# XiaoshuiHuang/IMFNet

Measured on AMD Instinct MI355X. Metric: descriptors/sec (32-D) on 3DMatch fragments, higher is better.
Workload: dtype f32 (bf16x3)

## Files before the change

### imfnet_amd/_lib.py

```python
import ctypes as C
import os

_HERE = os.path.dirname(os.path.abspath(__file__))
LIB_PATH = os.environ.get("IMF_LIB") or os.path.join(_HERE, "libimfnet_hip.so")

TILE_ROWS = 64
MASK_WORDS = 4
MAX_KVOL = 125
MAX_BATCH = 8
FLAG_RANGE = 32
XYZ_F32_QUOTIENT = 2
TAG_LABEL, TAG_REGS, TAG_WAVE8, TAG_WAVE4, TAG_HEAD, TAG_HALF, TAG_U48, TAG_OCC = 1, 2, 4, 8, 16, 64, 128, 256


class ImfError(RuntimeError):
    pass


class ConvArgs(C.Structure):
    _fields_ = [
        ("in_a", C.c_void_p), ("in_b", C.c_void_p),
        ("c_a", C.c_int32), ("c_b", C.c_int32),
        ("w_packed", C.c_void_p),
        ("kvol", C.c_int32), ("cout", C.c_int32),
# ... 219 lines not shown
    "imf_graph_end_capture": (_I, [_P, C.POINTER(C.c_void_p), C.POINTER(C.c_int)]),
    "imf_graph_abort_capture": (_I, [_P]),
    "imf_graph_launch": (_I, [_P, _P]),
    "imf_graph_destroy": (None, [_P]),
    "imf_pyramid_arena_bytes_caps": (_Z, [_L, _I, C.POINTER(C.c_int64)]),
    "imf_pyramid_build_dyn": (_I, [_P, _I, _P, _L, C.POINTER(C.c_int64), _D, _I, _P, _Z, _P, C.POINTER(LevelDesc), _P]),
    "imf_rulebook_conv_dyn": (_I, [_P, _L, _P, _L, _P, _I, _I, _P, _P, _P, _P]),
    "imf_rulebook_transpose_dyn": (_I, [_P, _L, _P, _L, _P, _I, _I, _P, _P, _P, _L, _P, _P]),
    "imf_conv_first_bitgrid_dyn": (_I, [_P, _L, _P, _P, _P, _I, _P, _Z, _P, _I, _P, _P, _I, _P, _P]),
    "imf_fusion_workspace_bytes_cap": (_Z, [_L]),
    "imf_fusion_attention_dyn": (_I, [_P, _L, _P, _P, _I, _P, C.POINTER(C.c_void_p), C.POINTER(C.c_void_p), _I, _I,
                                      C.POINTER(FusionWeights), C.c_float, _P, _P, _Z, _P]),
    "imf_fusion_attention_dyn_v": (_I, [_P, _L, _P, _P, _I, _P, C.POINTER(C.c_void_p), C.POINTER(C.c_void_p), _I, _I,
                                        C.POINTER(FusionWeights), C.c_float, _P, _P, _Z, _I, _P]),
    "imf_host_rigid_fit": (_I, [_P, _P, _I, _P]),
    "imf_ransac_workspace_bytes": (_Z, [_I]),
    "imf_ransac_registration": (_I, [_P, _L, _P, _L, _P, _I, _D, _D, _I, C.c_uint64, _P, _P, _P, _P, _Z, _P]),
    "imf_gather_points": (_I, [_P, _I, _P, _P, _L, _P, _P]),
    "imf_icp_workspace_bytes": (_Z, [_L, _L]),
    "imf_icp_point_to_point": (_I, [_P, _L, _P, _L, _D, _P, _I, _P, _P, _P, _P, _Z, _P]),
    "imf_icp_plane_workspace_bytes": (_Z, [_L, _L]),
    "imf_icp_point_to_plane": (_I, [_P, _L, _P, _P, _L, _D, _P, _I, _P, _P, _P, _P, _Z, _P]),
    "imf_normals_workspace_bytes": (_Z, [_L]),
    "imf_estimate_normals": (_I, [_P, _L, _I, _D, _P, _P, _P, _P, _P, _P, _Z, _P]),
    "imf_radius_count_workspace_bytes": (_Z, [_L]),
    "imf_radius_count": (_I, [_P, _L, _P, _L, _P, _D, _P, _P, _P, _P, _Z, _P]),
    "imf_radius_pairs_workspace_bytes": (_Z, [_L, _L]),
    "imf_radius_pairs": (_I, [_P, _L, _P, _L, _P, _D, _P, _P, _L, _P, _P, _P, _Z, _P]),
    "imf_robust_transform_workspace_bytes": (_Z, [_L]),
    "imf_robust_transform": (_I, [_P, _P, _P, _L, _P, _P, _P, _Z, _P]),
    "imf_tsdf_allocate_workspace_bytes": (_Z, [_L]),
    "imf_tsdf_allocate": (_I, [_P, _I, _P, C.POINTER(TsdfParams), _I, _P, _L, _P, _L, _P, _P, _Z, _P]),
    "imf_tsdf_integrate": (_I, [_P, _I, _P, C.POINTER(TsdfParams), _P, _P, _L, _P, _P]),
    "imf_tsdf_extract_workspace_bytes": (_Z, [_L]),
    "imf_tsdf_extract": (_I, [_P, _P, _P, _L, _P, _L, C.POINTER(TsdfParams), _P, _L, _P, _P, _Z, _P]),
    "imf_overlap_index_bytes": (_Z, [_L]),
    "imf_overlap_index_workspace_bytes": (_Z, [_L]),
    "imf_overlap_index_build": (_I, [_P, _L, _D, _P, _Z, C.POINTER(OverlapIndex), _P, _Z, _P]),
    "imf_overlap_bound": (_I, [_P, _P, _I, _L, _P, _P]),
    "imf_overlap_pair": (_I, [C.POINTER(OverlapIndex), C.POINTER(OverlapIndex), C.c_float, _L, _P, _P]),
    "imf_overlap_emit_workspace_bytes": (_Z, [_L]),
    "imf_overlap_emit": (_I, [_P, _L, _P, _P, _P, _Z, _P]),
    "imf_hash_capacity": (_L, [_L]),
    "imf_unique_workspace_bytes": (_Z, [_L]),
    "imf_voxelize": (_I, [_P, _I, _L, _D, _I, _P, _P, _P, _P, _L, _P, _P, _P]),
    "imf_downsample": (_I, [_P, _P, _L, _I, _P, _P, _P, _L, _P, _P]),
    "imf_pyramid_arena_bytes": (_Z, [_L, _I]),
    "imf_pyramid_build": (_I, [_P, _I, _L, _D, _I, _I, _P, _Z, _P, C.POINTER(LevelDesc), _P]),
    "imf_pyramid_build_batched": (_I, [_P, _I, _L, _D, C.POINTER(C.c_int64), _I, _I, _P, _Z, _P,
                                       C.POINTER(LevelDesc), _P]),
    "imf_rulebook_slots": (_L, [_L]),
    "imf_rulebook_conv": (_I, [_P, _L, _P, _L, _I, _I, _P, _P, _P, _P]),
    "imf_rulebook_sorted_workspace_bytes": (C.c_size_t, [_L]),
    "imf_rulebook_sort_by_occupancy": (_I, [_P, _I, _L, _L, _P, _P, _P, _P, _P, C.c_size_t, _P]),
    "imf_resunet_sorted_maps": (_I, [_I]),
    "imf_resunet_sorted_maps_n": (_I, [_I, _I]),
    "imf_rulebook_transpose_slots": (_L, [_L]),
    "imf_rulebook_transpose": (_I, [_P, _L, _P, _L, _I, _I, _P, _P, _P, _L, _P, _P]),
    "imf_packed_weight_floats": (_L, [_I, _I, _I]),
    "imf_packed_weight_floats_split16": (_L, [_I, _I, _I]),
    "imf_pack_weights": (_I, [_P, _I, _I, _I, _P, _P]),
    "imf_first_kernel_image_floats": (_L, [_I, _I]),
    "imf_pack_first_kernel": (_I, [_P, _I, _I, _P, _P]),
    "imf_pack_weights_split16": (_I, [_P, _I, _I, _I, _P, _P]),
    "imf_packed_weight_floats_bf16x3": (_L, [_I, _I, _I]),
    "imf_pack_weights_bf16x3": (_I, [_P, _I, _I, _I, _P, _P]),
    "imf_spconv_auto_split": (_I, [_L, _I, _I]),
    "imf_spconv_workspace_bytes": (_Z, [_L, _I, _I]),
    "imf_spconv_fwd": (_I, [C.POINTER(ConvArgs), _P]),
    "imf_pointwise_head": (_I, [C.POINTER(HeadArgs), _P]),
    "imf_spconv_small_cin": (_I, [_P, _I, _P, _I, _I, _P, _L, _L, _P, _P, _I, _P, _P]),
    "imf_fusion_workspace_bytes": (_Z, [_L]),
    "imf_fusion_attention_batched": (_I, [_P, _I, C.POINTER(C.c_int64), C.POINTER(C.c_int64), C.POINTER(C.c_void_p),
                                          C.POINTER(C.c_void_p), _I, _I, C.POINTER(FusionWeights), C.c_float, _P, _P,
                                          _Z, _P]),
    "imf_fusion_attention": (_I, [_P, _L, _P, _P, _I, _I, C.POINTER(FusionWeights), C.c_float, _P, _P, _Z, _P]),
    "imf_fusion_attention_batched_v": (_I, [_P, _I, C.POINTER(C.c_int64), C.POINTER(C.c_int64), C.POINTER(C.c_void_p),
                                            C.POINTER(C.c_void_p), _I, _I, C.POINTER(FusionWeights), C.c_float, _P, _P,
                                            _Z, _P, _I, _P]),
    "imf_image_workspace_bytes": (_Z, [_I, _I, _I]),
    "imf_image_tokens": (_I, [_I, _I]),
    "imf_image_tables_build": (_I, [_I, _I, _I, _P, _Z, _P]),
    "imf_image_branch": (_I, [C.POINTER(ImageDesc), _P, _I, _I, _I, _P, _Z, _P, _P, _P, _I, _P, _P]),
    "imf_image_train_tables_bytes": (_Z, [_I, _I, _I]),
    "imf_image_train_tables_build": (_I, [_I, _I, _I, _P, _Z, C.POINTER(ImageTrainTables), _P]),
    "imf_image_im2col7": (_I, [_P, _I, _I, _I, _P, _P]),
    "imf_image_maxpool_forward": (_I, [_P, _I, _I, _I, _I, _P, _P, _P]),
    "imf_image_maxpool_backward": (_I, [_P, _P, _I, _I, _I, _I, _P, _P]),
    "imf_conv_first_bitgrid_flags": (_I, [_P, _L, _P, _I, _P, _Z, _P, _I, _P, _P, _I, _P, _P, _P]),
    "imf_fusion_attention_batched_flags": (_I, [_P, _I, C.POINTER(C.c_int64), C.POINTER(C.c_int64), C.POINTER(C.c_void_p),
                                                C.POINTER(C.c_void_p), _I, _I, C.POINTER(FusionWeights), C.c_float, _P, _P,
                                                _Z, _P, _P]),
    "imf_bitgrid_words": (_Z, [_P, _I]),
    "imf_conv_first_bitgrid": (_I, [_P, _L, _P, _I, _P, _Z, _P, _I, _P, _P, _I, _P, _P]),
    "imf_conv_first_fused": (_I, [_P, _L, _P, _L, _I, _I, _P, _I, _P, _I, _P, _P, _I, _P, _P]),
}

_lib = None


def lib():
    global _lib
    if _lib is None:
        if not os.path.exists(LIB_PATH):
            raise ImfError(
                f"{LIB_PATH} not found: build it with `python -c 'import __graft_entry__ as g; g.build()'` "
                "or `make -C imfnet_amd/csrc`.  imfnet_amd has no CPU fallback.")
        handle = C.CDLL(LIB_PATH)
        for name, (res, args) in SIGNATURES.items():
            fn = getattr(handle, name)
            fn.restype, fn.argtypes = res, args
        _lib = handle
    return _lib


def check(rc, what):
    if rc != 0:
        msg = lib().imf_last_error().decode("utf-8", "replace")
        raise ImfError(f"{what} failed (rc={rc}): {msg}")
```

### imfnet_amd/csrc/image.hip

```cpp
#include <stdio.h>
#include <stdlib.h>
#include <string.h>

#include "common.h"
#include "image_shared.h"

namespace imf {
namespace {

constexpr int kC1 = 64, kC2 = 128, kKV = 256;

struct Plan {
  Table t4, t48, td, t8;
  float *im2col, *stem, *b4[3], *b8[4], *ln, *kv, *splitk;
  size_t splitk_bytes, total_bytes, table_bytes;
};

size_t splitk_need(int64_t n_out, int cout, int kvol) {
  const int64_t n_slots = imf_rulebook_slots(n_out);
  return imf_spconv_workspace_bytes(n_slots, cout, imf_spconv_auto_split(n_slots, cout, kvol));
}

Plan plan_of(const ImgShape &s, void *ws) {
  Plan p;
// ... 108 lines not shown
}

}
}

using namespace imf;

extern "C" {

size_t imf_image_workspace_bytes(int B, int H, int W) {
  if (B < 1 || H < 8 || W < 8) return 0;
  return plan_of(shape_of(B, H, W), nullptr).total_bytes + 256;
}

int imf_image_tokens(int H, int W) {
  const ImgShape s = shape_of(1, H, W);
  return s.H8 * s.W8;
}

int imf_image_tables_build(int B, int H, int W, void *workspace, size_t workspace_bytes, void *stream) {
  IMF_REQUIRE(workspace && B >= 1 && B <= IMF_MAX_BATCH && H >= 8 && W >= 8, "imf_image_tables_build: bad argument");
  IMF_REQUIRE(((uintptr_t)workspace & 255) == 0, "imf_image_tables_build: workspace must be 256-byte aligned");
  IMF_REQUIRE(workspace_bytes >= imf_image_workspace_bytes(B, H, W), "imf_image_tables_build: workspace too small");
  const ImgShape s = shape_of(B, H, W);
  const Plan p = plan_of(s, workspace);
  hipStream_t st = (hipStream_t)stream;
  IMF_CHECK_HIP(hipMemsetAsync(workspace, 0, p.table_bytes, st));
  auto build = [&](const Table &t, int Hin, int Win, int Hout, int Wout, int ksize, int stride, int pad) {
    k_img_rulebook<<<(unsigned)div_up(t.n_slots * t.kvol, 256), 256, 0, st>>>(
        s.B, Hin, Win, Hout, Wout, ksize, stride, pad, t.n_slots, t.tile_rows, t.nbr, t.tile_mask);
  };
  build(p.t4, s.H4, s.W4, s.H4, s.W4, 3, 1, 1);
  build(p.t48, s.H4, s.W4, s.H8, s.W8, 3, 2, 1);
  build(p.td, s.H4, s.W4, s.H8, s.W8, 1, 2, 0);
  build(p.t8, s.H8, s.W8, s.H8, s.W8, 3, 1, 1);
  IMF_CHECK_LAUNCH("k_img_rulebook");
  return IMF_OK;
}

int imf_image_branch(const imf_image_desc *net, const float *image, int B, int H, int W, void *workspace,
                     size_t workspace_bytes, float *feat_out, float *kt_packed, float *v_packed,
                     int tokens_padded, int32_t *flags, void *stream) {
  IMF_REQUIRE(net && image && workspace, "imf_image_branch: null pointer");
  IMF_REQUIRE(B >= 1 && B <= IMF_MAX_BATCH && H >= 8 && W >= 8, "imf_image_branch: B=%d H=%d W=%d", B, H, W);
  IMF_REQUIRE(((uintptr_t)workspace & 255) == 0, "imf_image_branch: workspace must be 256-byte aligned");
  IMF_REQUIRE(workspace_bytes >= imf_image_workspace_bytes(B, H, W), "imf_image_branch: workspace too small");
  IMF_REQUIRE(net->stem_w && net->stem_scale && net->stem_shift, "imf_image_branch: stem weights missing");
  for (int i = 0; i < 15; ++i)
    IMF_REQUIRE(net->conv[i].w_packed && net->conv[i].scale && net->conv[i].shift, "imf_image_branch: conv %d missing", i);
  const ImgShape s = shape_of(B, H, W);
  const int ntok = s.H8 * s.W8;
  const bool want_kv = kt_packed || v_packed;
  if (want_kv) {
    IMF_REQUIRE(kt_packed && v_packed && net->ln_g && net->ln_b && net->kv_w, "imf_image_branch: K/V outputs need ln / kv weights");
    IMF_REQUIRE(tokens_padded % 64 == 0 && tokens_padded >= ntok, "imf_image_branch: tokens_padded=%d for %d tokens",
                tokens_padded, ntok);
  }
  const Plan p = plan_of(s, workspace);
  hipStream_t st = (hipStream_t)stream;

  auto conv = [&](const imf_net_conv &c, const Table *t, int64_t n_rows, const float *in, const float *residual,
                  float *out) -> int {
    imf_conv_args a;
    memset(&a, 0, sizeof(a));
    a.in_a = in; a.c_a = c.cin; a.w_packed = c.w_packed; a.kvol = c.kvol; a.cout = c.cout;
    if (t) {
      IMF_REQUIRE(t->kvol == c.kvol, "imf_image_branch: kernel volume %d on a %d-tap table", c.kvol, t->kvol);
      a.tile_rows = t->tile_rows; a.nbr = t->nbr; a.tile_mask = t->tile_mask;
      a.n_slots = t->n_slots; a.n_out = t->n_out;
    } else {
      a.n_slots = imf_rulebook_slots(n_rows); a.n_out = n_rows;
    }
    a.scale = c.scale; a.shift = c.shift; a.residual = residual; a.relu = c.relu; a.out = out;
    a.variant = c.variant; a.split_k = 0;
    a.dyn_err = c.variant == 6 ? flags : nullptr;
    a.kernel_tag = IMF_TAG_LABEL;
    if (c.kvol == 9 && (c.variant == 6 || c.variant == 0 || c.variant == 3) && c.cout % 64 == 0) {
      a.kernel_tag |= IMF_TAG_WAVE8;
      a.split_k = 1;
    }
    a.workspace = p.splitk; a.workspace_bytes = p.splitk_bytes;
    return imf_spconv_fwd(&a, st);
  };

  {
    const int64_t total = s.n2 * kStemK;
    k_img_im2col7<<<(unsigned)div_up(total, 256), 256, 0, st>>>(image, B, H, W, s.H2, s.W2, p.im2col, net->variant == 6 ? flags : nullptr);
    IMF_CHECK_LAUNCH("k_img_im2col7");
    imf_net_conv c;
    memset(&c, 0, sizeof(c));
    c.w_packed = net->stem_w; c.kvol = 1; c.cin = kStemK; c.cout = kC1;
    c.scale = net->stem_scale; c.shift = net->stem_shift; c.relu = 1; c.variant = net->variant;
    int rc = conv(c, nullptr, s.n2, p.im2col, nullptr, p.stem);
    if (rc) return rc;
    const int64_t tot = s.n4 * (kC1 / 4);
    k_img_maxpool<<<(unsigned)div_up(tot, 256), 256, 0, st>>>(p.stem, B, s.H2, s.W2, s.H4, s.W4, kC1, p.b4[0]);
    IMF_CHECK_LAUNCH("k_img_maxpool");
  }
  int rc;
  int cur = 0;
  for (int blk = 0; blk < 3; ++blk) {
    const int mid = (cur + 1) % 3, nxt = (cur + 2) % 3;
    if ((rc = conv(net->conv[2 * blk], &p.t4, s.n4, p.b4[cur], nullptr, p.b4[mid]))) return rc;
    if ((rc = conv(net->conv[2 * blk + 1], &p.t4, s.n4, p.b4[mid], p.b4[cur], p.b4[nxt]))) return rc;
    cur = nxt;
  }
  if ((rc = conv(net->conv[6], &p.t48, s.n8, p.b4[cur], nullptr, p.b8[0]))) return rc;
  if ((rc = conv(net->conv[7], &p.td, s.n8, p.b4[cur], nullptr, p.b8[1]))) return rc;
  const bool last_is_out = feat_out != nullptr;
  if ((rc = conv(net->conv[8], &p.t8, s.n8, p.b8[0], p.b8[1], p.b8[2]))) return rc;
  int c8 = 2;
  for (int blk = 1; blk < 4; ++blk) {
    const int mid = (c8 + 1) % 4, nxt = (c8 + 2) % 4;
    float *dst = (blk == 3 && last_is_out) ? feat_out : p.b8[nxt];
    if ((rc = conv(net->conv[7 + 2 * blk], &p.t8, s.n8, p.b8[c8], nullptr, p.b8[mid]))) return rc;
    if ((rc = conv(net->conv[8 + 2 * blk], &p.t8, s.n8, p.b8[mid], p.b8[c8], dst))) return rc;
    c8 = nxt;
  }
  const float *feat = last_is_out ? feat_out : p.b8[c8];
  if (!want_kv) return IMF_OK;

  k_img_layernorm128<<<(unsigned)div_up(s.n8, 4), 256, 0, st>>>(feat, s.n8, net->ln_g, net->ln_b, p.ln, net->variant == 6 ? flags : nullptr);
  IMF_CHECK_LAUNCH("k_img_layernorm128");
  {
    imf_net_conv c;
    memset(&c, 0, sizeof(c));
    c.w_packed = net->kv_w; c.kvol = 1; c.cin = kC2; c.cout = kKV; c.variant = net->variant;
    if ((rc = conv(c, nullptr, s.n8, p.ln, nullptr, p.kv))) return rc;
  }
  const int64_t per2 = 2ll * 128 * tokens_padded;
  k_img_pack_kv<<<dim3((unsigned)div_up(per2, 256), (unsigned)B), 256, 0, st>>>(p.kv, ntok, tokens_padded, kt_packed,
                                                                              v_packed);
  IMF_CHECK_LAUNCH("k_img_pack_kv");
  return IMF_OK;
}

}
```

### imfnet_amd/csrc/image_shared.h

```cpp
#pragma once
#include "common.h"

namespace imf {
namespace {

struct ImgShape {
  int B, H, W;
  int H2, W2;
  int H4, W4;
  int H8, W8;
  int64_t n2, n4, n8;
};

ImgShape shape_of(int B, int H, int W) {
  ImgShape s;
  s.B = B; s.H = H; s.W = W;
  s.H2 = (H + 6 - 7) / 2 + 1; s.W2 = (W + 6 - 7) / 2 + 1;
  s.H4 = (s.H2 + 2 - 3) / 2 + 1; s.W4 = (s.W2 + 2 - 3) / 2 + 1;
  s.H8 = (s.H4 + 2 - 3) / 2 + 1; s.W8 = (s.W4 + 2 - 3) / 2 + 1;
  s.n2 = (int64_t)B * s.H2 * s.W2; s.n4 = (int64_t)B * s.H4 * s.W4; s.n8 = (int64_t)B * s.H8 * s.W8;
  return s;
}

constexpr int kStemK = 160;

struct Table {
  int32_t *tile_rows, *nbr;
  uint32_t *tile_mask;
  int64_t n_slots, n_out;
  int kvol;
};

size_t table_words(int64_t n_out, int kvol) {
  const int64_t n_slots = imf_rulebook_slots(n_out);
  return (size_t)n_slots * (1 + kvol) + (size_t)(n_slots / IMF_TILE_ROWS) * IMF_MASK_WORDS;
}

int32_t *place_table(Table &t, int32_t *p, int64_t n_out, int kvol) {
  t.n_out = n_out; t.kvol = kvol; t.n_slots = imf_rulebook_slots(n_out);
  t.tile_rows = p; p += t.n_slots;
  t.nbr = p; p += (size_t)kvol * t.n_slots;
  t.tile_mask = (uint32_t *)p; p += (size_t)(t.n_slots / IMF_TILE_ROWS) * IMF_MASK_WORDS;
  return p;
}

__global__ void __launch_bounds__(256)
k_img_rulebook(int B, int Hin, int Win, int Hout, int Wout, int ksize, int stride, int pad, int64_t n_slots,
               int32_t *__restrict__ tile_rows, int32_t *__restrict__ nbr, uint32_t *__restrict__ tile_mask) {
  const int64_t idx = (int64_t)blockIdx.x * blockDim.x + threadIdx.x;
  const int kvol = ksize * ksize;
  if (idx >= n_slots * kvol) return;
  const int k = (int)(idx / n_slots);
  const int64_t slot = idx - (int64_t)k * n_slots;
  const int64_t n_out = (int64_t)B * Hout * Wout;
  const int row = slot < n_out ? (int)slot : -1;
  if (k == 0) tile_rows[slot] = row;
  int found = -1;
  if (row >= 0) {
    const int b = row / (Hout * Wout), r = row - b * (Hout * Wout);
    const int oy = r / Wout, ox = r - oy * Wout;
    const int iy = oy * stride + k / ksize - pad, ix = ox * stride + k % ksize - pad;
    if (iy >= 0 && iy < Hin && ix >= 0 && ix < Win) found = (b * Hin + iy) * Win + ix;
  }
  nbr[idx] = found;
  const unsigned long long any = __ballot(found >= 0);
  if (any != 0ull && (threadIdx.x & 63) == 0)
    atomicOr(tile_mask + (slot >> 6) * IMF_MASK_WORDS + (k >> 5), 1u << (k & 31));
}

__global__ void __launch_bounds__(256)
k_img_im2col7(const float *__restrict__ img, int B, int H, int W, int Ho, int Wo, float *__restrict__ out,
              int32_t *flags) {
  const int64_t idx = (int64_t)blockIdx.x * blockDim.x + threadIdx.x;
  const int64_t total = (int64_t)B * Ho * Wo * kStemK;
  if (idx >= total) return;
  const int c = (int)(idx % kStemK);
  const int64_t row = idx / kStemK;
  float v = 0.f;
  if (c < 147) {
    const int tap = c / 3, ch = c - 3 * tap, ky = tap / 7, kx = tap - 7 * ky;
    const int b = (int)(row / (Ho * Wo)), r = (int)(row - (int64_t)b * Ho * Wo);
    const int oy = r / Wo, ox = r - oy * Wo;
    const int iy = 2 * oy + ky - 3, ix = 2 * ox + kx - 3;
    if (iy >= 0 && iy < H && ix >= 0 && ix < W) v = img[(((int64_t)b * 3 + ch) * H + iy) * W + ix];
  }
  if (flags && !(fabsf(v) < 65504.f)) atomicOr(flags, 32);
// ... 6 lines not shown
```

### imfnet_amd/ops.py

```python
import ctypes as C
import os
import weakref

import torch

from . import _lib
from ._lib import ConvArgs, HeadArgs, ImfError, LevelDesc, TILE_ROWS, MASK_WORDS, check


TRACE = None


class _Ev:

    def __init__(self):
        L = _lib.lib()
        self.begin, self.end = L.imf_event_create(), L.imf_event_create()

    def elapsed_ms(self):
        return _lib.lib().imf_event_elapsed_ms(self.begin, self.end)

    def __del__(self):
        try:
            L = _lib.lib()
# ... 971 lines not shown
    shapes = ((n, cu), (n, cs), (cu + cs, ch), (ch, co), (1, co))
    names = ("du", "ds", "dw1", "dw2", "dbias")
    for name, t, shape in (("dy", dy, (n, co)), ("h", h, (n, ch))) + ((("y", y, (n, co)), ("r", r, (n,))) if normalize else ()):
        if tuple(_req(t, torch.float32, name).shape) != shape or t.device != u.device:
            raise ImfError(f"{name} must be {shape} on {u.device}")
    if outputs is None:
        want = [True] * 5 if want is None else list(want)
        outputs = [torch.empty(shape, dtype=torch.float32, device=u.device) if k else None for shape, k in zip(shapes, want)]
    else:
        for name, t, shape in zip(names, outputs, shapes):
            if t is not None and (tuple(_req(t, torch.float32, name).shape) != shape or t.device != u.device):
                raise ImfError(f"{name} must be {shape} on {u.device}")
    L = _lib.lib()
    nbytes = L.imf_head_train_workspace_bytes(n)
    ws = torch.empty(max(nbytes // 4, 4), dtype=torch.float32, device=u.device)
    meta = torch.zeros(1, dtype=torch.int32, device=u.device)
    check(L.imf_head_train_backward(_ptr(dy), _ptr(y) if normalize else None, _ptr(r) if normalize else None, _ptr(h),
                                    _ptr(u), cu, _ptr(s), cs, n, w1.data_ptr(), ch, w2.data_ptr(), co,
                                    int(bool(normalize)), *[_ptr(t) for t in outputs], ws.data_ptr(), nbytes,
                                    meta.data_ptr(), _stream()), "imf_head_train_backward")
    return (*outputs, meta)


TRAIN_IMAGE_CHOICES = ("torch", "hip")
TRAIN_IMAGE = os.environ.get("IMF_TRAIN_IMAGE", "torch")
if TRAIN_IMAGE not in TRAIN_IMAGE_CHOICES:
    raise ImfError(f"IMF_TRAIN_IMAGE={TRAIN_IMAGE!r}: one of {', '.join(TRAIN_IMAGE_CHOICES)}")


def set_train_image(name):
    global TRAIN_IMAGE
    if name not in TRAIN_IMAGE_CHOICES:
        raise ImfError(f"image kernels {name!r}: one of {', '.join(TRAIN_IMAGE_CHOICES)}")
    prev, TRAIN_IMAGE = TRAIN_IMAGE, name
    return prev


def image_trunk_shapes(H, W):
    down = lambda v, k, p: (v + 2 * p - k) // 2 + 1
    h2, w2 = down(H, 7, 3), down(W, 7, 3)
    h4, w4 = down(h2, 3, 1), down(w2, 3, 1)
    return (h2, w2), (h4, w4), (down(h4, 3, 1), down(w4, 3, 1))


class ImageTrainTables:

    def __init__(self, B, H, W, device):
        L = _lib.lib()
        nbytes = L.imf_image_train_tables_bytes(B, H, W)
        if nbytes == 0:
            raise ImfError(f"image tables: B={B} H={H} W={W} (B >= 1, H and W >= 8)")
        self.B, self.H, self.W = B, H, W
        self.shapes = image_trunk_shapes(H, W)
        self.storage = torch.empty(nbytes, dtype=torch.uint8, device=device)
        c = _lib.ImageTrainTables()
        with torch.cuda.device(self.storage.device):
            check(L.imf_image_train_tables_build(B, H, W, self.storage.data_ptr(), nbytes, C.byref(c), _stream()),
                  "imf_image_train_tables_build")
        base = self.storage.data_ptr()

        def view(addr, words):
            off = addr - base
            return self.storage[off:off + 4 * words].view(torch.int32)

        for name in _lib.IMAGE_TRAIN_TABLES:
            t = getattr(c, name)
            setattr(self, name, Rulebook(view(t.tile_rows, t.n_slots), view(t.nbr, t.kvol * t.n_slots),
                                         view(t.tile_mask, t.n_slots // TILE_ROWS * MASK_WORDS), t.n_slots, t.n_out, t.kvol))
        self.stem = rulebook_identity(B * self.shapes[0][0] * self.shapes[0][1], device)


def image_im2col7(image):
    _req(image, torch.float32, "image", 4)
    B, ch, H, W = image.shape
    if ch != 3:
        raise ImfError(f"image must be [B,3,H,W], got {tuple(image.shape)}")
    (h2, w2), _, _ = image_trunk_shapes(H, W)
    out = torch.empty((B * h2 * w2, 160), dtype=torch.float32, device=image.device)
    with torch.cuda.device(image.device):
        check(_lib.lib().imf_image_im2col7(image.data_ptr(), B, H, W, out.data_ptr(), _stream()), "imf_image_im2col7")
    return out


def _pool_rows(t, dtype, name, rows, c):
    _req(t, dtype, name, 2)
    if tuple(t.shape) != (rows, c):
        raise ImfError(f"{name} must be [{rows}, {c}], got {tuple(t.shape)}")
    return t


def image_maxpool_forward(x, B, Hin, Win):
    c = x.shape[1] if torch.is_tensor(x) and x.dim() == 2 else 0
    _pool_rows(x, torch.float32, "x", B * Hin * Win, c)
    rows = B * ((Hin - 1) // 2 + 1) * ((Win - 1) // 2 + 1)
    out = torch.empty((rows, c), dtype=torch.float32, device=x.device)
    tap = torch.empty((rows, c), dtype=torch.uint8, device=x.device)
    with torch.cuda.device(x.device):
        check(_lib.lib().imf_image_maxpool_forward(x.data_ptr(), B, Hin, Win, c, out.data_ptr(), tap.data_ptr(), _stream()),
              "imf_image_maxpool_forward")
    return out, tap


def image_maxpool_backward(dout, tap, B, Hin, Win, din=None):
    c = dout.shape[1] if torch.is_tensor(dout) and dout.dim() == 2 else 0
    rows = B * ((Hin - 1) // 2 + 1) * ((Win - 1) // 2 + 1)
    _pool_rows(dout, torch.float32, "dout", rows, c)
    _pool_rows(tap, torch.uint8, "tap", rows, c)
    if din is None:
        din = torch.empty((B * Hin * Win, c), dtype=torch.float32, device=dout.device)
    else:
        _pool_rows(din, torch.float32, "din", B * Hin * Win, c)
    with torch.cuda.device(dout.device):
        check(_lib.lib().imf_image_maxpool_backward(dout.data_ptr(), tap.data_ptr(), B, Hin, Win, c, din.data_ptr(),
                                                    _stream()), "imf_image_maxpool_backward")
    return din


def dam_heat(out_prenorm, hidden, targets, accumulate=True, n_dev=None, heat=None):
    _req(out_prenorm, torch.float32, "out_prenorm", 2)
    _req(hidden, torch.float32, "hidden", 2)
    _req(targets, torch.int32, "targets", 1)
    n, c_out = out_prenorm.shape
    c_hid = hidden.shape[1]
    if hidden.shape[0] != n:
        raise ImfError(f"hidden must have {n} rows, got {hidden.shape[0]}")
    if c_out != 32 or c_hid < 32 or c_hid % 32:
        raise ImfError(f"DAM supports c_out = 32 and c_hid a positive multiple of 32, got c_out={c_out} c_hid={c_hid}")
    T = targets.shape[0]
    if n_dev is not None:
        _req(n_dev, torch.int32, "n_dev")
    dev = out_prenorm.device
    if heat is None:
        heat = torch.empty((T, n), dtype=torch.float32, device=dev)
    elif tuple(_req(heat, torch.float32, "heat", 2).shape) != (T, n):
        raise ImfError(f"heat must be [{T}, {n}], got {tuple(heat.shape)}")
    minmax = torch.zeros((T, 2), dtype=torch.float32, device=dev)
    flags = torch.zeros(T, dtype=torch.int32, device=dev)
    weights = torch.zeros((T, 32), dtype=torch.float32, device=dev)
    if T:
        check(_lib.lib().imf_dam_heat(out_prenorm.data_ptr(), n, _ptr(n_dev), hidden.data_ptr(), c_hid, c_out,
                                      targets.data_ptr(), T, int(bool(accumulate)), weights.data_ptr(), heat.data_ptr(),
                                      minmax.data_ptr(), flags.data_ptr(), _stream()), "imf_dam_heat")
    return heat, minmax, flags, weights


TRAIN_OPTIM_CHOICES = ("torch", "hip")
TRAIN_OPTIM = os.environ.get("IMF_TRAIN_OPTIM", "torch")
if TRAIN_OPTIM not in TRAIN_OPTIM_CHOICES:
    raise ImfError(f"IMF_TRAIN_OPTIM={TRAIN_OPTIM!r}: one of {', '.join(TRAIN_OPTIM_CHOICES)}")


def set_train_optim(name):
    global TRAIN_OPTIM
    if name not in TRAIN_OPTIM_CHOICES:
        raise ImfError(f"optim kernels {name!r}: one of {', '.join(TRAIN_OPTIM_CHOICES)}")
    prev, TRAIN_OPTIM = TRAIN_OPTIM, name
    return prev


class WeightImages:
    __slots__ = ("ref", "shape", "fwd", "bwd", "flip", "version", "key")

    def __init__(self, param, fwd, bwd, flip):
        self.ref, self.shape, self.fwd, self.bwd, self.flip = weakref.ref(param), tuple(param.shape), fwd, bwd, bool(flip)
        self.version, self.key = -1, None

# ... 72 lines not shown
```

### include/imfnet_hip.h

```cpp
#ifndef IMFNET_HIP_H
#define IMFNET_HIP_H

#include <stddef.h>
#include <stdint.h>

#ifdef __cplusplus
extern "C" {
#endif

#define IMF_OK            0
#define IMF_EINVAL       -1
#define IMF_ELAUNCH      -2
#define IMF_EUNSUPPORTED -3

#define IMF_TILE_ROWS    64
#define IMF_MAX_KVOL     125
#define IMF_MAX_BATCH    8
#define IMF_MASK_WORDS   4
#define IMF_XYZ_F32_QUOTIENT 2

int imf_version(void);
const char *imf_last_error(void);

typedef struct imf_slot {
// ... 133 lines not shown

typedef struct imf_head_args {
  const float *in_a;
  const float *in_b;
  int32_t c_a, c_b;
  const float *w1_packed;
  const float *scale1, *shift1;
  int32_t relu1, c_mid;
  const float *w2_packed;
  const float *scale2, *shift2;
  int32_t l2norm, c_out;
  int64_t n;
  const int32_t *n_dev;
  float *out;
  int32_t *flags;
  void *ev_begin, *ev_end;
  int32_t a_split;
  int32_t variant;
} imf_head_args;
int imf_pointwise_head(const imf_head_args *args , void *stream);

int imf_spconv_small_cin(const float *in, int cin, const float *w, int kvol, int cout,
                         const int32_t *nbr, int64_t n_slots, int64_t n_out,
                         const float *scale, const float *shift, int relu,
                         float *out, void *stream);

int imf_conv_first_fused(const imf_slot *table, int64_t capacity,
                         const int32_t *coords, int64_t n, int ts, int ksize, const float *in, int cin,
                         const float *w , int cout,
                         const float *scale, const float *shift, int relu, float *out, void *stream);

size_t imf_bitgrid_words(const int32_t *bbox , int ksize);
int imf_conv_first_bitgrid(const int32_t *coords, int64_t n, const int32_t *bbox , int ksize,
                           uint32_t *grid, size_t grid_words, const float *w ,
                           int cout, const float *scale, const float *shift, int relu, float *out,
                           void *stream);

int imf_conv_first_bitgrid_flags(const int32_t *coords, int64_t n, const int32_t *bbox , int ksize,
                                 uint32_t *grid, size_t grid_words, const float *w, int cout, const float *scale,
                                 const float *shift, int relu, float *out, int32_t *flags, void *stream);
int imf_conv_first_bitgrid_dyn(const int32_t *coords, int64_t n_cap, const int32_t *n_dev, const int32_t *bbox_dev,
                               int32_t *err, int ksize, uint32_t *grid, size_t grid_words, const float *w, int cout,
                               const float *scale, const float *shift, int relu, float *out, void *stream);

typedef struct imf_fusion_weights {
  const float *ln1_g, *ln1_b, *wq_p, *wo_p, *bo, *ln2_g, *ln2_b, *w1_p, *b1, *w2_p, *b2;
  const float *w1_f32, *w2_f32;
} imf_fusion_weights;
size_t imf_fusion_workspace_bytes(int64_t n);
int imf_fusion_attention(const float *x, int64_t n, const float *kt_packed, const float *v_packed,
                         int n_tokens, int tokens_padded, const imf_fusion_weights *w ,
                         float scale, float *out, void *workspace, size_t workspace_bytes, void *stream);
int imf_fusion_attention_batched(const float *x, int n_items, const int64_t *item_row0, const int64_t *item_rows,
                                 const float *const *kt_packed, const float *const *v_packed, int n_tokens,
                                 int tokens_padded, const imf_fusion_weights *w , float scale, float *out,
                                 void *workspace, size_t workspace_bytes, void *stream);
int imf_fusion_attention_batched_v(const float *x, int n_items, const int64_t *item_row0, const int64_t *item_rows,
                                   const float *const *kt_packed, const float *const *v_packed, int n_tokens,
                                   int tokens_padded, const imf_fusion_weights *w , float scale, float *out,
                                   void *workspace, size_t workspace_bytes, int32_t *flags, int variant, void *stream);

typedef struct imf_net_conv {
  const float *w_packed;
  int32_t kvol, cin, cout;
  const float *scale, *shift;
  int32_t relu, l2norm, variant;
} imf_net_conv;

typedef struct imf_image_desc {
  const float *stem_w, *stem_scale, *stem_shift;
  imf_net_conv conv[15];
  const float *ln_g, *ln_b;
  const float *kv_w;
  int32_t variant;
} imf_image_desc;

size_t imf_image_workspace_bytes(int B, int H, int W);
int imf_image_tokens(int H, int W);
int imf_image_tables_build(int B, int H, int W, void *workspace, size_t workspace_bytes, void *stream);
int imf_image_branch(const imf_image_desc *net , const float *image, int B, int H, int W,
                     void *workspace, size_t workspace_bytes, float *feat_out, float *kt_packed,
                     float *v_packed, int tokens_padded, int32_t *flags ,
                     void *stream);

typedef struct imf_image_table {
  int32_t *tile_rows, *nbr;
  uint32_t *tile_mask;
  int64_t n_slots, n_out;
  int32_t kvol;
} imf_image_table;
typedef struct imf_image_train_tables {
  imf_image_table t4, t48, t48T, td, tdT, t8;
} imf_image_train_tables;
size_t imf_image_train_tables_bytes(int B, int H, int W);
int imf_image_train_tables_build(int B, int H, int W, void *storage, size_t storage_bytes,
                                 imf_image_train_tables *out , void *stream);
int imf_image_im2col7(const float *image_nchw, int B, int H, int W, float *out, void *stream);
int imf_image_maxpool_forward(const float *in, int B, int Hin, int Win, int C, float *out, uint8_t *tap, void *stream);
int imf_image_maxpool_backward(const float *dout, const uint8_t *tap, int B, int Hin, int Win, int C, float *din,
                               void *stream);

int imf_fusion_attention_batched_flags(const float *x, int n_items, const int64_t *item_row0, const int64_t *item_rows,
                                       const float *const *kt_packed, const float *const *v_packed, int n_tokens,
                                       int tokens_padded, const imf_fusion_weights *w , float scale,
                                       float *out, void *workspace, size_t workspace_bytes, int32_t *flags, void *stream);
size_t imf_fusion_workspace_bytes_cap(int64_t n_cap);
int imf_fusion_attention_dyn(const float *x, int64_t n_cap, const int32_t *n_dev, const int32_t *item_starts_dev,
                             int n_items, int32_t *err, const float *const *kt_packed, const float *const *v_packed,
                             int n_tokens, int tokens_padded, const imf_fusion_weights *w , float scale,
                             float *out, void *workspace, size_t workspace_bytes, void *stream);
int imf_fusion_attention_dyn_v(const float *x, int64_t n_cap, const int32_t *n_dev, const int32_t *item_starts_dev,
                               int n_items, int32_t *err, const float *const *kt_packed, const float *const *v_packed,
                               int n_tokens, int tokens_padded, const imf_fusion_weights *w , float scale,
                               float *out, void *workspace, size_t workspace_bytes, int variant, void *stream);


typedef struct imf_resunet_desc {
  int32_t channels[5], tr_channels[5];
  int32_t in_channels, out_channels, first_ksize;
  int32_t small_first;
  imf_net_conv conv[23];
  const float *first_kernel, *first_scale, *first_shift;
  imf_fusion_weights fusion;
  float fusion_scale;
  const float *first_kernel_image;
} imf_resunet_desc;
int64_t imf_first_kernel_image_floats(int kvol, int cout);
int imf_pack_first_kernel(const float *w , int kvol, int cout, float *image, void *stream);

typedef struct imf_net_trace {
  void *ev_begin, *ev_end;
  const int32_t *nbr;
  int32_t kvol, cin, cout, split;
  int64_t n_slots, n_out;
  int32_t launched;
  int32_t level, slots_extra;
  int32_t kernel_tag;
} imf_net_trace;

int imf_resunet_conv_kernel_tag(int level, int kvol, int cin, int cout, int variant, int n_items);
int imf_resunet_sorted_maps(int variant);
int imf_resunet_sorted_maps_n(int variant, int n_items);

typedef struct imf_resunet_io {
  imf_level level[4];
  int64_t n[4];
  const int32_t *bbox;
  const float *x;
  int32_t x_all_ones;
  int32_t n_items;
  int64_t item_row0[IMF_MAX_BATCH];
  int64_t item_rows[IMF_MAX_BATCH];
  const float *kt_packed[IMF_MAX_BATCH], *v_packed[IMF_MAX_BATCH];
  int32_t n_tokens, tokens_padded;
  void *image_ready;
  void *fusion_done;
  void *int_arena;  size_t int_arena_bytes;
  void *float_arena; size_t float_arena_bytes;
  float *out;
  void *events[16];
  void *side_stream, *main_stream;
  imf_net_trace *trace;
  int32_t dyn;
  const int32_t *meta;
  size_t bitgrid_words;
  const void *pyramid;
// ... 286 lines not shown
```

Baseline: 92.69 million.

## Add dense 3x3 image conv kernel replacing sparse rulebook convs in image trunk

Adds a dedicated dense 3x3 convolution kernel for the image branch. It computes neighbour addresses directly from the pixel grid and does not go through rulebook tables. Operands are loaded straight into LDS with buffer loads, the math uses bf16x3 MFMA, and scale/shift/residual/relu are fused into the epilogue. The image trunk's 3x3 convs use it by default when variant is 3, unless IMF_IMAGE_DENSE=0. This removes the neighbour-table indirection and tile-mask overhead of the sparse path, at the cost of a new hand-scheduled kernel with a 4-wave cross-wave reduction and no split-K.

```diff
diff --git a/imfnet_amd/_lib.py b/imfnet_amd/_lib.py
--- a/imfnet_amd/_lib.py
+++ b/imfnet_amd/_lib.py
@@ -325,6 +325,7 @@
     "imf_image_tokens": (_I, [_I, _I]),
     "imf_image_tables_build": (_I, [_I, _I, _I, _P, _Z, _P]),
     "imf_image_branch": (_I, [C.POINTER(ImageDesc), _P, _I, _I, _I, _P, _Z, _P, _P, _P, _I, _P, _P]),
+    "imf_image_conv3x3": (_I, [_P, _I, _I, _I, _I, _I, _I, _P, _P, _P, _P, _I, _P, _P]),
     "imf_image_train_tables_bytes": (_Z, [_I, _I, _I]),
     "imf_image_train_tables_build": (_I, [_I, _I, _I, _P, _Z, C.POINTER(ImageTrainTables), _P]),
     "imf_image_im2col7": (_I, [_P, _I, _I, _I, _P, _P]),
diff --git a/imfnet_amd/csrc/image.hip b/imfnet_amd/csrc/image.hip
--- a/imfnet_amd/csrc/image.hip
+++ b/imfnet_amd/csrc/image.hip
@@ -214,6 +214,13 @@
     a.workspace = p.splitk; a.workspace_bytes = p.splitk_bytes;
     return imf_spconv_fwd(&a, st);
   };
+  const bool dense = image_dense_enabled();
+  auto conv3 = [&](const imf_net_conv &c, const Table *t, int Hin, int Win, int stride, int64_t n_rows, const float *in,
+                   const float *residual, float *out) -> int {
+    if (dense && c.variant == 3 && c.kvol == 9 && (c.cin == kC1 || c.cin == kC2) && (c.cout == kC1 || c.cout == kC2))
+      return imf_image_conv3x3(in, s.B, Hin, Win, stride, c.cin, c.cout, c.w_packed, c.scale, c.shift, residual, c.relu, out, st);
+    return conv(c, t, n_rows, in, residual, out);
+  };
 
   {
     const int64_t total = s.n2 * kStemK;
@@ -233,20 +240,20 @@
   int cur = 0;
   for (int blk = 0; blk < 3; ++blk) {
     const int mid = (cur + 1) % 3, nxt = (cur + 2) % 3;
-    if ((rc = conv(net->conv[2 * blk], &p.t4, s.n4, p.b4[cur], nullptr, p.b4[mid]))) return rc;
-    if ((rc = conv(net->conv[2 * blk + 1], &p.t4, s.n4, p.b4[mid], p.b4[cur], p.b4[nxt]))) return rc;
+    if ((rc = conv3(net->conv[2 * blk], &p.t4, s.H4, s.W4, 1, s.n4, p.b4[cur], nullptr, p.b4[mid]))) return rc;
+    if ((rc = conv3(net->conv[2 * blk + 1], &p.t4, s.H4, s.W4, 1, s.n4, p.b4[mid], p.b4[cur], p.b4[nxt]))) return rc;
     cur = nxt;
   }
-  if ((rc = conv(net->conv[6], &p.t48, s.n8, p.b4[cur], nullptr, p.b8[0]))) return rc;
+  if ((rc = conv3(net->conv[6], &p.t48, s.H4, s.W4, 2, s.n8, p.b4[cur], nullptr, p.b8[0]))) return rc;
   if ((rc = conv(net->conv[7], &p.td, s.n8, p.b4[cur], nullptr, p.b8[1]))) return rc;
   const bool last_is_out = feat_out != nullptr;
-  if ((rc = conv(net->conv[8], &p.t8, s.n8, p.b8[0], p.b8[1], p.b8[2]))) return rc;
+  if ((rc = conv3(net->conv[8], &p.t8, s.H8, s.W8, 1, s.n8, p.b8[0], p.b8[1], p.b8[2]))) return rc;
   int c8 = 2;
   for (int blk = 1; blk < 4; ++blk) {
     const int mid = (c8 + 1) % 4, nxt = (c8 + 2) % 4;
     float *dst = (blk == 3 && last_is_out) ? feat_out : p.b8[nxt];
-    if ((rc = conv(net->conv[7 + 2 * blk], &p.t8, s.n8, p.b8[c8], nullptr, p.b8[mid]))) return rc;
-    if ((rc = conv(net->conv[8 + 2 * blk], &p.t8, s.n8, p.b8[mid], p.b8[c8], dst))) return rc;
+    if ((rc = conv3(net->conv[7 + 2 * blk], &p.t8, s.H8, s.W8, 1, s.n8, p.b8[c8], nullptr, p.b8[mid]))) return rc;
+    if ((rc = conv3(net->conv[8 + 2 * blk], &p.t8, s.H8, s.W8, 1, s.n8, p.b8[mid], p.b8[c8], dst))) return rc;
     c8 = nxt;
   }
   const float *feat = last_is_out ? feat_out : p.b8[c8];
diff --git a/imfnet_amd/csrc/image_conv.hip b/imfnet_amd/csrc/image_conv.hip
--- /dev/null
+++ b/imfnet_amd/csrc/image_conv.hip
@@ -0,0 +1,214 @@
+#include <stdlib.h>
+
+#include "spconv_shared.h"
+
+namespace imf {
+namespace {
+
+struct DenseConvParams {
+  const float *in, *w, *scale, *shift, *residual;
+  float *out;
+  int Hin, Win, Hout, Wout, stride, cout, relu;
+  int n_out;
+  unsigned in_bytes, w_bytes;
+};
+
+constexpr unsigned kOutside = 0xF0000000u;
+
+template <int NCC, int RB>
+__global__ void __launch_bounds__(256, 3)
+k_img_conv3x3(const DenseConvParams p) {
+  constexpr int W = 4, NSUB = 9 * NCC, UR = 16 * RB;
+  constexpr unsigned SUB_BYTES = 12288u;
+  constexpr int PART_F4 = 144;
+  constexpr int REG_F4 = 128 * RB > PART_F4 ? 128 * RB : PART_F4;
+  __shared__ float4 smem[W * REG_F4];
+
+  const int y = blockIdx.y >> 1, half = blockIdx.y & 1;
+  const int row0 = blockIdx.x * UR;
+  if (row0 >= p.n_out) return;
+  const int tid = threadIdx.x, lane = tid & 63, r16 = lane & 15, q4 = lane >> 4;
+  const int wave = __builtin_amdgcn_readfirstlane(tid >> 6);
+
+  const int row_w = lane >> 2;
+  const unsigned wr_byte = 16u * (unsigned)((lane & 3) ^ ((4 - (row_w >> 2)) & 3));
+  const int rd_slot = 4 * r16 + (q4 ^ ((4 - (r16 >> 2)) & 3));
+  float4 *const areg = smem + wave * REG_F4;
+
+  const int hw = p.Hout * p.Wout;
+  int iy0[RB], ix0[RB], ctr[RB];
+#pragma unroll
+  for (int b = 0; b < RB; ++b) {
+    const int pix = row0 + 16 * b + row_w;
+    iy0[b] = ix0[b] = -4;
+    ctr[b] = 0;
+    if (pix < p.n_out) {
+      const int img = pix / hw, r = pix - img * hw;
+      const int oy = r / p.Wout, ox = r - oy * p.Wout;
+      iy0[b] = oy * p.stride;
+      ix0[b] = ox * p.stride;
+      ctr[b] = (img * p.Hin + iy0[b]) * p.Win + ix0[b];
+    }
+  }
+
+  const __amdgpu_buffer_rsrc_t rs_w = __builtin_amdgcn_make_buffer_rsrc(const_cast<float *>(p.w), (short)0, (int)p.w_bytes, 0x00020000);
+  const __amdgpu_buffer_rsrc_t rs_a = __builtin_amdgcn_make_buffer_rsrc(const_cast<float *>(p.in), (short)0, (int)p.in_bytes, 0x00020000);
+  const unsigned stride_a = (unsigned)NCC * 128u;
+  const unsigned whalf = ((unsigned)y * (unsigned)NSUB * 2u + (unsigned)half) * 6144u;
+  const unsigned woff = (unsigned)lane * 16u;
+
+#define IMF_D_DMA_ROWS(t, live)                                                                                    \
+  {                                                                                                                \
+    const int k_ = (t) / NCC, ky_ = k_ / 3;                                                                        \
+    const int dy_ = ky_ - 1, dx_ = k_ - 3 * ky_ - 1;                                                               \
+    const unsigned soff = (unsigned)((t) % NCC) << 7;                                                              \
+    _Pragma("unroll") for (int b_ = 0; b_ < RB; ++b_) {                                                            \
+      const bool in_ = (live) && (unsigned)(iy0[b_] + dy_) < (unsigned)p.Hin && (unsigned)(ix0[b_] + dx_) < (unsigned)p.Win; \
+      const unsigned voff = (in_ ? (unsigned)(ctr[b_] + dy_ * p.Win + dx_) * stride_a : kOutside) + wr_byte;       \
+      __builtin_amdgcn_raw_ptr_buffer_load_lds(rs_a, (lds_void *)(areg + 128 * b_), 16, voff, soff, 0, 0);         \
+      __builtin_amdgcn_raw_ptr_buffer_load_lds(rs_a, (lds_void *)(areg + 128 * b_ + 64), 16, voff + 64u, soff, 0, 0); \
+    }                                                                                                              \
+  }
+#define IMF_D_LD_W(dst, t)                                                                                         \
+  {                                                                                                                \
+    const unsigned wso = whalf + (unsigned)(t) * SUB_BYTES;                                                        \
+    _Pragma("unroll") for (int cb_ = 0; cb_ < 2; ++cb_)                                                            \
+        _Pragma("unroll") for (int h_ = 0; h_ < 3; ++h_)                                                           \
+            (dst)[cb_][h_] = __builtin_bit_cast(bf16x8,                                                            \
+                __builtin_amdgcn_raw_buffer_load_b128(rs_w, woff, wso + 1024u * (unsigned)(3 * cb_ + h_), 0));     \
+  }
+
+  f32x4 acc[RB][2];
+#pragma unroll
+  for (int b = 0; b < RB; ++b)
+#pragma unroll
+    for (int cb = 0; cb < 2; ++cb) acc[b][cb] = (f32x4){0.f, 0.f, 0.f, 0.f};
+
+  const int t0 = wave * NSUB / W, t1 = (wave + 1) * NSUB / W;
+  bf16x8 wX[2][3], wY[2][3];
+#define IMF_D_TERM(I, J)                                                                                 \
+  _Pragma("unroll") for (int b = 0; b < RB; ++b)                                                         \
+      _Pragma("unroll") for (int cb = 0; cb < 2; ++cb)                                                   \
+          acc[b][cb] = __builtin_amdgcn_mfma_f32_16x16x32_bf16(ap[b][I], BP[cb][J], acc[b][cb], 0, 0, 0);
+#define IMF_D_STAGE(t)                                                                                             \
+  {                                                                                                                \
+    const bool more = (t) + 1 < t1;                                                                                \
+    const int tn = more ? (t) + 1 : (t);                                                                           \
+    IMF_D_LD_W(NXT, tn)                                                                                            \
+    asm volatile("s_waitcnt vmcnt(6)" ::: "memory");                        \
+    float4 a0[RB], a1[RB];                                                                                         \
+    _Pragma("unroll") for (int b = 0; b < RB; ++b) {                                                               \
+      a0[b] = lds_read16(&areg[128 * b + rd_slot]);                                                                \
+      a1[b] = lds_read16(&areg[128 * b + 64 + rd_slot]);                                                           \
+    }                                                                                                              \
+    asm volatile("s_waitcnt lgkmcnt(0)" ::: "memory");                                 \
+    IMF_D_DMA_ROWS(tn, more)                                                                                       \
+    __builtin_amdgcn_sched_barrier(0);                                                                             \
+    bf16x8 ap[RB][3];                                                                                              \
+    _Pragma("unroll") for (int b = 0; b < RB; ++b) split_b3(a0[b], a1[b], ap[b][0], ap[b][1], ap[b][2]);           \
+    IMF_B3_TERMS(IMF_D_TERM)                                                                                       \
+    __builtin_amdgcn_sched_barrier(0);                                                                             \
+  }
+  IMF_D_DMA_ROWS(t0, true)
+  __builtin_amdgcn_sched_barrier(0);
+  IMF_D_LD_W(wX, t0)
+  __builtin_amdgcn_sched_barrier(0);
+#pragma unroll 1
+  for (int t = t0;;) {
+#define BP wX
+#define NXT wY
+    IMF_D_STAGE(t)
+#undef BP
+#undef NXT
+    if (++t >= t1) break;
+#define BP wY
+#define NXT wX
+    IMF_D_STAGE(t)
+#undef BP
+#undef NXT
+    if (++t >= t1) break;
+  }
+  asm volatile("s_waitcnt vmcnt(0)" ::: "memory");
+#undef IMF_D_STAGE
+#undef IMF_D_TERM
+#undef IMF_D_LD_W
+#undef IMF_D_DMA_ROWS
+
+#pragma unroll
+  for (int b = 0; b < RB; ++b) {
+    if (b) __syncthreads();
+    float *const mine = reinterpret_cast<float *>(areg);
+#pragma unroll
+    for (int cb = 0; cb < 2; ++cb)
+#pragma unroll
+      for (int r = 0; r < 4; ++r) mine[(4 * q4 + r) * 36 + 16 * cb + r16] = acc[b][cb][r];
+    __syncthreads();
+    if (tid >= 128) continue;
+    const int lrow = tid >> 3, c4 = tid & 7;
+    const int phys = lrow * 9 + c4;
+    float4 s = lds_read16(&smem[phys]);
+#pragma unroll
+    for (int w = 1; w < W; ++w) {
+      const float4 v = lds_read16(&smem[w * REG_F4 + phys]);
+      s.x += v.x; s.y += v.y; s.z += v.z; s.w += v.w;
+    }
+    const int orow = row0 + 16 * b + lrow;
+    if (orow >= p.n_out) continue;
+    const int col = y * 64 + half * 32 + 4 * c4;
+    float4 sc = make_float4(1.f, 1.f, 1.f, 1.f), sh = make_float4(0.f, 0.f, 0.f, 0.f);
+    if (p.scale) sc = *reinterpret_cast<const float4 *>(p.scale + col);
+    if (p.shift) sh = *reinterpret_cast<const float4 *>(p.shift + col);
+    s.x = s.x * sc.x + sh.x; s.y = s.y * sc.y + sh.y;
+    s.z = s.z * sc.z + sh.z; s.w = s.w * sc.w + sh.w;
+    if (p.residual) {
+      const float4 rr = *reinterpret_cast<const float4 *>(p.residual + (long long)orow * p.cout + col);
+      s.x += rr.x; s.y += rr.y; s.z += rr.z; s.w += rr.w;
+    }
+    if (p.relu) { s.x = fmaxf(s.x, 0.f); s.y = fmaxf(s.y, 0.f); s.z = fmaxf(s.z, 0.f); s.w = fmaxf(s.w, 0.f); }
+    *reinterpret_cast<float4 *>(p.out + (long long)orow * p.cout + col) = s;
+  }
+}
+
+int dense_env() {
+  static const int v = [] {
+    const char *e = getenv("IMF_IMAGE_DENSE");
+    return e ? atoi(e) : -1;
+  }();
+  return v;
+}
+
+}
+
+bool image_dense_enabled() { return dense_env() != 0; }
+
+}
+
+using namespace imf;
+
+extern "C" int imf_image_conv3x3(const float *in, int B, int H, int W, int stride, int cin, int cout, const float *w_packed,
+                                 const float *scale, const float *shift, const float *residual, int relu, float *out,
+                                 void *stream) {
+  IMF_REQUIRE(in && w_packed && out, "imf_image_conv3x3: null pointer");
+  IMF_REQUIRE(B >= 1 && H >= 1 && W >= 1 && (stride == 1 || stride == 2), "imf_image_conv3x3: B=%d H=%d W=%d stride=%d", B, H, W, stride);
+  IMF_REQUIRE((cin == 64 || cin == 128) && (cout == 64 || cout == 128), "imf_image_conv3x3: cin=%d cout=%d (64 or 128 each)", cin, cout);
+  IMF_REQUIRE(aligned16(in) && aligned16(w_packed) && aligned16(out) && aligned16(scale) && aligned16(shift) && aligned16(residual),
+              "imf_image_conv3x3: pointers must be 16-byte aligned");
+  const int Hout = (H - 1) / stride + 1, Wout = (W - 1) / stride + 1;
+  const int64_t in_bytes = (int64_t)B * H * W * cin * 4, n_out = (int64_t)B * Hout * Wout;
+  IMF_REQUIRE(in_bytes < 0x70000000ll, "imf_image_conv3x3: input of %lld bytes (must stay below 1.75 GiB)", (long long)in_bytes);
+  DenseConvParams p;
+  p.in = in; p.w = w_packed; p.scale = scale; p.shift = shift; p.residual = residual; p.out = out;
+  p.Hin = H; p.Win = W; p.Hout = Hout; p.Wout = Wout; p.stride = stride; p.cout = cout; p.relu = relu;
+  p.n_out = (int)n_out;
+  p.in_bytes = (unsigned)in_bytes;
+  p.w_bytes = (unsigned)(cout / 64) * 9u * (unsigned)(cin / 32) * 12288u;
+  const int rb = dense_env() == 32 ? 2 : 1;
+  const dim3 grid((unsigned)div_up(n_out, 16 * rb), (unsigned)(cout / 32), 1);
+  hipStream_t st = (hipStream_t)stream;
+  if (cin == 64 && rb == 1) k_img_conv3x3<2, 1><<<grid, 256, 0, st>>>(p);
+  else if (cin == 64) k_img_conv3x3<2, 2><<<grid, 256, 0, st>>>(p);
+  else if (rb == 1) k_img_conv3x3<4, 1><<<grid, 256, 0, st>>>(p);
+  else k_img_conv3x3<4, 2><<<grid, 256, 0, st>>>(p);
+  IMF_CHECK_LAUNCH("k_img_conv3x3");
+  return IMF_OK;
+}
diff --git a/imfnet_amd/csrc/image_shared.h b/imfnet_amd/csrc/image_shared.h
--- a/imfnet_amd/csrc/image_shared.h
+++ b/imfnet_amd/csrc/image_shared.h
@@ -2,6 +2,9 @@
 #include "common.h"
 
 namespace imf {
+
+bool image_dense_enabled();
+
 namespace {
 
 struct ImgShape {
diff --git a/imfnet_amd/ops.py b/imfnet_amd/ops.py
--- a/imfnet_amd/ops.py
+++ b/imfnet_amd/ops.py
@@ -1077,6 +1077,29 @@
     return out
 
 
+def image_conv3x3(x, B, H, W, w_packed, cout, stride=1, scale=None, shift=None, residual=None, relu=False, out=None):
+    cin = x.shape[1] if torch.is_tensor(x) and x.dim() == 2 else 0
+    _pool_rows(x, torch.float32, "x", B * H * W, cin)
+    _req(w_packed, torch.float32, "w_packed", 1)
+    need = _lib.lib().imf_packed_weight_floats_bf16x3(9, cin, cout) if cin % 32 == 0 and cout % 32 == 0 and cin and cout else 0
+    if not need or w_packed.numel() < need:
+        raise ImfError(f"w_packed has {w_packed.numel()} floats, the bf16x3 image of [9, {cin}, {cout}] needs {need}")
+    rows = B * ((H - 1) // stride + 1) * ((W - 1) // stride + 1) if stride in (1, 2) else 0
+    for t, name in ((scale, "scale"), (shift, "shift")):
+        if t is not None and (_req(t, torch.float32, name, 1).numel() != cout):
+            raise ImfError(f"{name} must have {cout} values")
+    if residual is not None:
+        _pool_rows(residual, torch.float32, "residual", rows, cout)
+    if out is None:
+        out = torch.empty((rows, cout), dtype=torch.float32, device=x.device)
+    else:
+        _pool_rows(out, torch.float32, "out", rows, cout)
+    with torch.cuda.device(x.device):
+        check(_lib.lib().imf_image_conv3x3(x.data_ptr(), B, H, W, stride, cin, cout, w_packed.data_ptr(), _ptr(scale), _ptr(shift),
+                                           _ptr(residual), int(bool(relu)), out.data_ptr(), _stream()), "imf_image_conv3x3")
+    return out
+
+
 def _pool_rows(t, dtype, name, rows, c):
     _req(t, dtype, name, 2)
     if tuple(t.shape) != (rows, c):
diff --git a/include/imfnet_hip.h b/include/imfnet_hip.h
--- a/include/imfnet_hip.h
+++ b/include/imfnet_hip.h
@@ -239,6 +239,9 @@
                      void *workspace, size_t workspace_bytes, float *feat_out, float *kt_packed,
                      float *v_packed, int tokens_padded, int32_t *flags ,
                      void *stream);
+int imf_image_conv3x3(const float *in, int B, int H, int W, int stride, int cin, int cout, const float *w_packed,
+                      const float *scale, const float *shift, const float *residual, int relu, float *out,
+                      void *stream);
 
 typedef struct imf_image_table {
   int32_t *tile_rows, *nbr;
```

Result: slower. 91.27 million (-1.5%).
